# amin-abouee/semi-direct-visual-odometry

Hardware: AMD Instinct MI355X
Metric: frame-pair alignments/sec @2000 feats, 5-lvl pyramid; SE(3) err vs ref (higher is better)
Workload: dtype f64

## Files before the change

### semi-direct-visual-odometry_amd/csrc/align_refv.hip

```cpp
#include "svo_internal.h"
#include "svo_math.h"
#include "svo_wave.h"
#include "ref_common.h"

#include <utility>

namespace svo {
#if defined(SVO_TIMELINE)
SVO_TL_DEFINE(k2v)
SVO_TL_READER(k2v)
#endif


namespace {

using namespace refsel;

constexpr int kVT = 512;
constexpr int kVW = kVT / 64;
#ifndef SVO_ONEWAVE
#define SVO_ONEWAVE 2048
#endif
constexpr int kRowPad = 128;

#include "refv_rows.h"

template <class G, int R, uint32_t MB, bool PRE, uint32_t OW>
struct Lay {
    using Rows = G;
    static constexpr int kRows = R;
    static constexpr int kRegRows = G::kRegRows;
    static constexpr uint32_t kMbCap = MB;
    static constexpr bool kPreload = PRE;
    static constexpr uint32_t kCap = (uint32_t)R * kVT;
    static constexpr uint32_t kOneWave = OW;
    static constexpr uint32_t kStage = 2 * OW;
    static_assert(OW % 256 == 0 && OW / 64 <= G::kRegRows && OW <= 4096, "one-wave rows: register quads of wave 0");
    static_assert(R > G::kRegRows && R <= kRowPad, "rows");
    static_assert(2 * OW <= MB && MB % 64 == 0, "one-wave segment and its mailbox");
    static_assert(!PRE || kStage + 64 * G::kRegRows <= MB, "staging of wave 0's rows inside the mailbox");
    static_assert(!PRE || R % (kVW - 1) == 0, "stage_wave0 covers every row");
};
#ifndef SVO_ONEWAVE_A
#define SVO_ONEWAVE_A SVO_ONEWAVE
#endif
using LayA = Lay<RowsA, 98, 12288, true, SVO_ONEWAVE_A>;
using LayB = Lay<RowsB, 118, 4352, false, SVO_ONEWAVE>;
using LayC = Lay<RowsC, 128, 1344, false, 512>;
using LayADbg = Lay<RowsA, 98, 12288, true, 1024>;
using LayBDbg = Lay<RowsB, 118, 4352, false, 1024>;

template <class L>
struct VShared {
    double mbx[L::kMbCap + 64];
    uint32_t rec[4][kVW][kRowPad];
    uint32_t cnt[kVW][kRowPad];
    double pub[6];
    uint32_t pubk[4];
    double bcd;
    uint32_t srch[4];
    double lrow[L::kRows - L::kRegRows][kVT];
    uint32_t tmp[2 * kVW];
};
static_assert(sizeof(VShared<LayC>) <= 163840, "LayC's shared state fits the CU's LDS");

struct VDiag {
    uint32_t nblock[2], nwave[2], heap[2], nchunk[2];
    uint64_t cyc[2];
    uint64_t ph[12];
    uint32_t nlog;
#if defined(SVO_STAMPS_WAVES)
    union {
        uint32_t log[64][2];
        uint32_t phw[kVW][12];
    };
#else
    uint32_t log[64][2];
#endif
    double* tr;
    uint32_t trcap, ntr;
};
constexpr uint32_t kTrHead = 8;
#if defined(SVO_STAMPS_SMALL)
[[maybe_unused]] constexpr bool kStampsSmall = true;
#else
[[maybe_unused]] constexpr bool kStampsSmall = false;
#endif
#if defined(SVO_STAMPS) && defined(SVO_STAMPS_WAVES)
#define VSTAMP(i) \
    do { \
        if (kStampOn && dg) { \
            const uint64_t t_ = clock64(); \
            if (!kStampsSmall || small_round) phacc[i] += (uint32_t)(t_ - tstamp); \
            tstamp = t_; \
        } \
    } while (0)
#elif defined(SVO_STAMPS)
#define VSTAMP(i) \
    do { \
        if (kStampOn && dg && tid == 0) { \
            const uint64_t t_ = clock64(); \
            if (!kStampsSmall || small_round) dg->ph[i] += t_ - tstamp; \
            tstamp = t_; \
        } \
    } while (0)
#else
#define VSTAMP(i) \
    do { \
        (void)tstamp; \
    } while (0)
#endif

__device__ __forceinline__ uint32_t lane_sel(uint64_t m, uint32_t a, uint32_t b) {
    uint32_t r;
    asm("v_cndmask_b32_e64 %0, %2, %1, %3" : "=v"(r) : "v"(a), "v"(b), "s"(m));
    return r;
}
__device__ __forceinline__ uint32_t lane_put(uint32_t x, uint32_t v, uint32_t j, uint32_t me) {
    uint32_t r;
    uint64_t eq;
    asm("v_cmp_eq_u32_e64 %1, %2, %3\n\tv_cndmask_b32_e64 %0, %4, %5, %1"
        : "=v"(r), "=&s"(eq)
        : "v"(me), "s"(j), "v"(x), "v"(v));
    return r;
}
template <class L>
struct VSel {
    using G = typename L::Rows;
    static constexpr int R = L::kRows;
    static constexpr int kVRegRows = L::kRegRows;
    static constexpr int kGenQuads = G::kGenQuads;
    static constexpr uint32_t kMbCap = L::kMbCap;
    static constexpr uint32_t kOneWave = L::kOneWave;
    static constexpr uint32_t kStage = L::kStage;
    static constexpr int kQuads = (R + 3) / 4;
#ifndef SVO_FEWROWS
#define SVO_FEWROWS 8
#endif
    static constexpr int kFewRows = SVO_FEWROWS;
    static constexpr bool kChunkSteps = kMbCap < 12288;
#ifndef SVO_QG
#define SVO_QG 4
#endif
    static constexpr int kQG = SVO_QG;
    static constexpr bool kStampOn = L::kPreload;
    static __device__ __forceinline__ double vget(int r) { return G::vget(r); }
    static __device__ __forceinline__ void vset(int r, double x) { G::vset(r, x); }
    static __device__ __forceinline__ uint64_t vcmp_ge(int r, double p) { return G::vcmp_ge(r, p); }
    static __device__ __forceinline__ uint64_t vcmp_le(int r, double p) { return G::vcmp_le(r, p); }
    static __device__ __forceinline__ void vsel(int r, double x, uint64_t m) { G::vsel(r, x, m); }
    VShared<L>& sh;
    double* gseg;
    uint32_t gdummy;
    VDiag* dg;
    uint32_t M, nth;
    int tid, lane, wave;
    uint32_t f, l;
    uint32_t xk0 = 0, xk1 = 0;
    int depth;
    bool rec;
    double lo_val;
    int P;
    bool small_round = false;
#if defined(SVO_STAMPS) && defined(SVO_STAMPS_WAVES)
    uint32_t phacc[12] = {};
#endif

    template <bool kWrite, typename F>
    __device__ __forceinline__ void rows(int rlo, int rhi, F&& body) {
        const int r1 = rhi < kVRegRows - 1 ? rhi : kVRegRows - 1;
        for (int r = rlo; r <= r1; ++r) {
            double x = vget(r);
            body(r, x);
            if (kWrite) vset(r, x);
        }
#pragma unroll 2
        for (int r = rlo > kVRegRows ? rlo : kVRegRows; r <= rhi; ++r) {
            double& y = sh.lrow[r - kVRegRows][tid];
            double x = y;
            body(r, x);
            if (kWrite) y = x;
        }
    }
    __device__ __forceinline__ double row_val(int r) const {
        return r < kVRegRows ? vget(r) : sh.lrow[r - kVRegRows][tid];
    }
    __device__ __forceinline__ void row_set(int r, uint32_t ln, double x) {
        if ((uint32_t)lane != ln) return;
        if (r < kVRegRows) vset(r, x);
        else sh.lrow[r - kVRegRows][tid] = x;
    }
    __device__ __forceinline__ void load_raw(const double* src) {
        constexpr int kL = R - kVRegRows;
        if constexpr (kL <= 12) {
            double x[kL];
#pragma unroll
            for (int i = 0; i < kL; ++i) {
                const uint32_t q = (uint32_t)(kVRegRows + i) * kVT + (uint32_t)tid;
                x[i] = __builtin_nontemporal_load(src + (q < M ? q : 0u));
            }
            G::load(src, M * 8u, tid);
#pragma unroll
            for (int i = 0; i < kL; ++i) {
                const uint32_t q = (uint32_t)(kVRegRows + i) * kVT + (uint32_t)tid;
                sh.lrow[i][tid] = q < M ? x[i] : 0.0;
            }
        } else {
            G::load(src, M * 8u, tid);
#pragma unroll 2
            for (int r = kVRegRows; r < R; ++r) {
                const uint32_t q = (uint32_t)r * kVT + (uint32_t)tid;
                sh.lrow[r - kVRegRows][tid] = q < M ? src[q] : 0.0;
            }
        }
    }
    __device__ __forceinline__ void stage_wave0(const double* src) {
        double* const stg = sh.mbx + kStage;
#pragma unroll
        for (int i = 0; i < R / (kVW - 1); ++i) {
            const int r = wave - 1 + (kVW - 1) * i;
            const uint32_t q = (uint32_t)r * kVT + (uint32_t)lane;
            const double x = q < M ? src[q] : 0.0;
            if (r < kVRegRows) stg[64 * r + lane] = x;
            else sh.lrow[r - kVRegRows][lane] = x;
        }
    }
    __device__ __forceinline__ void unstage_wave0() {
        const uint32_t a = (uint32_t)(uintptr_t)(sh.mbx + kStage) + 8u * (uint32_t)lane;
        G::unstage(a);
    }
    __device__ __forceinline__ void load(const double* src, bool mad, double med, bool preloaded) {
        if (!preloaded) load_raw(src);
        if (mad) {
            const uint64_t mb = uni(__builtin_bit_cast(uint64_t, med));
            G::mad(mb);
            rows<true>(kVRegRows, R - 1, [&](int, double& x) __attribute__((always_inline)) { x = fabs(x - med); });
        }
    }
    __device__ __forceinline__ void wave_rows(uint32_t s0, uint32_t s1, int& rlo, int& rhi) const {
        const int w = wave;
        rlo = (int)s0 <= w ? 0 : ((int)s0 - w + kVW - 1) / kVW;
        rhi = (int)s1 < w ? -1 : ((int)s1 - w) / kVW;
    }
    static __device__ __forceinline__ uint64_t row_mask(int fw, int lw, int r) {
        const int b = r * kVT;
        const int lo = fw - b, hi = lw - b;
        return low_mask((uint32_t)(hi < 0 ? 0 : hi)) & ~low_mask((uint32_t)(lo < 0 ? 0 : lo));
    }
    __device__ __forceinline__ void publish(uint32_t q, int slot) {
        if (((q >> 6) & (kVW - 1)) != (uint32_t)wave) return;
        const double x = row_val((int)(q >> 9));
        if ((uint32_t)lane == (q & 63u)) sh.pub[slot] = x;
    }
    __device__ __forceinline__ void dump(double* dst, uint32_t dbase, double* dummy) {
        int rlo, rhi;
        wave_rows(f >> 6, (l - 1) >> 6, rlo, rhi);
        const int fo = (int)f - tid, lo = (int)l - tid;
        double* const d = dst + ((uint32_t)tid - dbase);
        double* const dl = dummy + lane;
        rows<false>(rlo, rhi, [&](int r, double x) __attribute__((always_inline)) {
            const int b = r * kVT;
            *(b >= fo && b < lo ? d + b : dl) = x;
        });
    }

    struct WaveRows {
        int rlo, rhi;
        uint64_t ge_first, le_first, last;
    };
    __device__ __forceinline__ WaveRows wave_segment(uint32_t s0, uint32_t s1) const {
        WaveRows w;
        wave_rows(s0, s1, w.rlo, w.rhi);
        const int fw = (int)f - 64 * wave, lw = (int)l - 64 * wave;
        w.le_first = row_mask(fw, lw, w.rlo);
        w.last = row_mask(fw, lw, w.rhi);
        const bool own_f = ((f >> 6) & (kVW - 1)) == (uint32_t)wave && (int)(f >> 9) == w.rlo;
        w.ge_first = w.le_first & ~(own_f ? 1ull << (f & 63u) : 0ull);
        return w;
    }
    static __device__ __forceinline__ void opaque(int& a, int& b) { asm volatile("" : "+s"(a), "+s"(b)); }
    template <int Q>
    __device__ __forceinline__ void cls_quad(double p, int rlo, int rhi, uint32_t (&acc)[2][4]) {
        opaque(rlo, rhi);
        if (4 * Q + 3 < rlo || 4 * Q > rhi) return;
        cls_quad_in<Q>(p, acc);
    }
    template <int Q>
    __device__ __forceinline__ void cls_quad_in(double p, uint32_t (&acc)[2][4]) {
        constexpr int g = (4 * Q) >> 6;
        if constexpr (Q < kGenQuads) {
            G::template cls4<Q>(p, acc[g]);
        } else {
#pragma unroll
            for (int i = 0; i < 4; ++i) {
                const int r = 4 * Q + i;
                if (r >= R) continue;
                const double x = sh.lrow[r - kVRegRows][tid];
                const uint64_t ge = __ballot(!(x < p)), le = __ballot(!(p < x));
                acc[g][0] = lane_write(acc[g][0], (uint32_t)ge, (uint32_t)(r & 63));
                acc[g][1] = lane_write(acc[g][1], (uint32_t)(ge >> 32), (uint32_t)(r & 63));
                acc[g][2] = lane_write(acc[g][2], (uint32_t)le, (uint32_t)(r & 63));
                acc[g][3] = lane_write(acc[g][3], (uint32_t)(le >> 32), (uint32_t)(r & 63));
            }
        }
    }
    template <int Gq, int... Is>
    __device__ __forceinline__ void cls_group(double p, int rlo, int rhi, uint32_t (&acc)[2][4],
                                              std::integer_sequence<int, Is...>) {
        opaque(rlo, rhi);
        constexpr int r0 = 4 * kQG * Gq, r1 = r0 + 4 * (int)sizeof...(Is) - 1;
        if (r1 < rlo || r0 > rhi) return;
        if (r0 >= rlo && r1 <= rhi) (cls_quad_in<kQG * Gq + Is>(p, acc), ...);
        else (cls_quad<kQG * Gq + Is>(p, rlo, rhi, acc), ...);
    }
    template <int... Gs>
    __device__ __forceinline__ void cls_quads(double p, int rlo, int rhi, uint32_t (&acc)[2][4],
                                              std::integer_sequence<int, Gs...>) {
        (cls_group<Gs>(p, rlo, rhi, acc, std::make_integer_sequence<int, (kQuads - kQG * Gs < kQG ? kQuads - kQG * Gs : kQG)>{}), ...);
    }
    __device__ __forceinline__ void cls_rows(double p, int rlo, int rhi, uint32_t (&acc)[2][4]) {
        for (int r = rlo; r <= rhi; ++r) {
            uint64_t ge, le;
            if (r < kVRegRows) {
                G::vcmp2(r, p, ge, le);
            } else {
                const double x = sh.lrow[r - kVRegRows][tid];
                ge = __ballot(!(x < p));
                le = __ballot(!(p < x));
            }
            const bool mine = lane == (r & 63);
#pragma unroll
            for (int g = 0; g < 2; ++g) {
                if (g != (r >> 6)) continue;
                acc[g][0] = mine ? (uint32_t)ge : acc[g][0];
// ... 52 lines not shown
                own += v < wave ? C.c[g][v] : 0u;
                t += C.c[g][v];
            }
            rt[g] = t;
            C.pw[g] = own;
        }
        const uint32_t i0 = wave_incl_scan(rt[0]);
        const uint32_t t0 = uni(lane_read(i0, 63));
        const uint32_t i1 = wave_incl_scan(rt[1]) + t0;
        C.rp[0] = i0 - rt[0];
        C.rp[1] = i1 - rt[1];
        C.pw[0] += C.rp[0];
        C.pw[1] += C.rp[1];
        const uint32_t tot = uni(lane_read(i1, 63));
        C.totG = tot & 0xFFFFu;
        C.totL = tot >> 16;
    }
    template <int G>
    __device__ __forceinline__ uint32_t step_pre_g(const Ctl& C, uint32_t ln, uint32_t v) const {
        uint32_t pk = uni(lane_read(C.rp[G], (int)ln));
#pragma unroll
        for (int u = 0; u < kVW; ++u)
            if ((uint32_t)u < v) pk += uni(lane_read(C.c[G][u], (int)ln));
        return pk;
    }
    __device__ __forceinline__ uint32_t step_pre(const Ctl& C, uint32_t s) const {
        const uint32_t r = s >> 3, v = s & (kVW - 1);
        return r < 64 ? step_pre_g<0>(C, r, v) : step_pre_g<1>(C, r - 64, v);
    }
    static __device__ __forceinline__ uint32_t kval(uint32_t pk, int kind) {
        return kind == 0 ? pk & 0xFFFFu : kind == 1 ? pk >> 16 : (pk & 0xFFFFu) + (pk >> 16);
    }
    template <int G>
    __device__ __forceinline__ uint32_t walk_row(const Ctl& C, uint32_t ln, int kind, uint32_t rank, uint32_t& pre) const {
        uint32_t pk = uni(lane_read(C.rp[G], (int)ln)), s = 0, p0 = pk;
#pragma unroll
        for (int u = 0; u < kVW; ++u) {
            if (kval(pk, kind) < rank) { s = (uint32_t)u; p0 = pk; }
            pk += uni(lane_read(C.c[G][u], (int)ln));
        }
        pre = p0;
        return (64u * G + ln) * kVW + s;
    }
    __device__ __forceinline__ uint32_t find_step(const Ctl& C, int kind, uint32_t rank, uint32_t& pre) const {
        const uint32_t n = popc(__ballot(kval(C.rp[0], kind) < rank)) + popc(__ballot(kval(C.rp[1], kind) < rank));
        const uint32_t jr = n - 1u;
        return jr < 64 ? walk_row<0>(C, jr, kind, rank, pre) : walk_row<1>(C, jr - 64, kind, rank, pre);
    }
    __device__ __forceinline__ uint64_t rec_mask(uint32_t s, int kind) const {
        const uint32_t r = s >> 3, v = s & (kVW - 1);
        return ((uint64_t)uni(sh.rec[2 * kind + 1][v][r]) << 32) | uni(sh.rec[2 * kind][v][r]);
    }
    __device__ __forceinline__ uint32_t locate(const Ctl& C, int kind, uint32_t rank) const {
        uint32_t pre;
        const uint32_t s = find_step(C, kind, rank, pre);
        return s * 64u + wave_select_bit(rec_mask(s, kind), rank - kval(pre, kind) - 1u);
    }
    __device__ __forceinline__ uint32_t locate_lds(const Ctl& C, int kind, uint32_t rank) const {
        const uint32_t n = popc(__ballot(kval(C.rp[0], kind) < rank)) + popc(__ballot(kval(C.rp[1], kind) < rank));
        const uint32_t jr = n - 1u, g = jr >> 6, ln = jr & 63u;
        uint32_t pk = uni(lane_read(g ? C.rp[1] : C.rp[0], (int)ln)), st = 0, p0 = pk;
#pragma unroll
        for (int u = 0; u < kVW; ++u) {
            if (kval(pk, kind) < rank) { st = (uint32_t)u; p0 = pk; }
            pk += uni(sh.cnt[u][jr]);
        }
        const uint32_t s = jr * kVW + st;
        return s * 64u + wave_select_bit(rec_mask(s, kind), rank - kval(p0, kind) - 1u);
    }
    __device__ __forceinline__ uint32_t wave_select_bit(uint64_t m, uint32_t j) const {
        const uint64_t hit = __ballot(((m >> lane) & 1ull) && lanes_below(m) == j);
        return (uint32_t)__builtin_ctzll(hit);
    }
    __device__ __forceinline__ uint32_t wave_crossing_ks(uint32_t gcar, uint32_t lcar, uint64_t ge, uint64_t le) const {
        const uint32_t me = (uint32_t)lane;
        const uint32_t g = gcar + lanes_below(ge) + (uint32_t)((ge >> me) & 1ull);
        const uint32_t lc = lcar - (lanes_below(le) + (uint32_t)((le >> me) & 1ull));
        const uint64_t q = __ballot(g >= lc);
        const uint32_t lo = q ? (uint32_t)__builtin_ctzll(q) + 1u : 64u;
        const uint32_t g1 = gcar + popc(ge & low_mask(lo - 1));
        const uint32_t l2 = lcar - popc(le & low_mask(lo));
        return g1 > l2 ? g1 : l2;
    }
    __device__ __forceinline__ void publish_cand(const Ctl& C, uint32_t q, int i, uint32_t ks, int side) {
        if (((q >> 6) & (kVW - 1)) != (uint32_t)wave) return;
        const double x = row_val((int)(q >> 9));
        uint32_t k = 0;
        if (ks) {
            const uint32_t s = q >> 6, b = q & 63u, r = s >> 3;
            const uint64_t m = rec_mask(s, side);
            if ((m >> b) & 1ull) {
                const uint32_t pp = r < 64 ? uni(lane_read(C.pw[0], (int)r)) : uni(lane_read(C.pw[1], (int)(r - 64)));
                const uint32_t below = popc(m & low_mask(b));
                k = side ? C.totL - ((pp >> 16) + below) : (pp & 0xFFFFu) + below + 1u;
                if (k > ks) k = 0;
            }
        }
        if ((uint32_t)lane == (q & 63u)) {
            sh.pub[i] = x;
            sh.pubk[i] = k;
        }
    }

    template <bool kWrite>
    __device__ __forceinline__ void generic_row(const Ctl& C, int side, int r, uint64_t gm, double p, uint32_t k0,
                                                uint32_t k1, bool chunked) {
        const uint32_t pp = r < 64 ? uni(lane_read(C.pw[0], r)) : uni(lane_read(C.pw[1], r - 64));
        const uint32_t nk = k1 - k0;
        const uint32_t b = side == 0 ? (pp & 0xFFFFu) - k0 : C.totL - 1u - k0 - (pp >> 16);
        double* const mbx = sh.mbx;
        const uint32_t dslot = kMbCap + (uint32_t)lane;
        uint64_t m;
        double x = 0.0;
        const bool reg = r < kVRegRows;
        if (!reg) x = sh.lrow[r - kVRegRows][tid];
        if (chunked) m = rec_mask((uint32_t)(r * kVW + wave), side);
        else if (side == 0) m = reg ? vcmp_ge(r, p) : __ballot(!(x < p));
        else m = reg ? vcmp_le(r, p) : __ballot(!(p < x));
        m &= gm;
        const uint32_t kk = side == 0 ? b + lanes_below(m) : b - lanes_below(m);
        const uint64_t okm = m & __ballot(kk < nk);
        const uint32_t a = lane_sel(okm, kk, dslot);
        if (kWrite) {
            mbx[a] = reg ? vget(r) : x;
        } else {
            const double t = mbx[a];
            if (reg) vsel(r, t, okm);
            else if ((okm >> lane) & 1ull) sh.lrow[r - kVRegRows][tid] = t;
        }
    }
    template <int Q, bool kWrite, int S>
    __device__ __forceinline__ void ex_quad(const Ctl& C, double p, int ra, int rb, const uint32_t (&pb)[2]) {
        opaque(ra, rb);
        if (4 * Q + 3 < ra || 4 * Q > rb) return;
        constexpr int g = (4 * Q) >> 6;
        if constexpr (Q < kGenQuads) {
            if (4 * Q >= ra && 4 * Q + 3 <= rb) {
                if (kWrite) G::template src4<Q, S>(p, pb[g]);
                else G::template tgt4<Q, S>(p, pb[g]);
            } else {
                if (kWrite) G::template src4e<Q, S>(p, pb[g], (uint32_t)ra, (uint32_t)(rb - ra));
                else G::template tgt4e<Q, S>(p, pb[g], (uint32_t)ra, (uint32_t)(rb - ra));
            }
        } else {
#pragma unroll
            for (int i = 0; i < 4; ++i) {
                const int r = 4 * Q + i;
                if (r < R && r >= ra && r <= rb) generic_row<kWrite>(C, S, r, ~0ull, p, xk0, xk1, false);
            }
        }
    }
    template <int Q, bool kWrite, int S>
    __device__ __forceinline__ void ex_quad_in(const Ctl& C, double p, const uint32_t (&pb)[2]) {
        constexpr int g = (4 * Q) >> 6;
        if constexpr (Q < kGenQuads) {
            if (kWrite) G::template src4<Q, S>(p, pb[g]);
            else G::template tgt4<Q, S>(p, pb[g]);
        } else {
#pragma unroll
            for (int i = 0; i < 4; ++i) {
                const int r = 4 * Q + i;
                if (r < R) generic_row<kWrite>(C, S, r, ~0ull, p, xk0, xk1, false);
            }
        }
    }
    template <bool kWrite, int S>
    __device__ __forceinline__ void ex_quads(const Ctl& C, double p, int ra, int rb, uint32_t k0) {
        const uint32_t mb = (uint32_t)(uintptr_t)sh.mbx - 8u * k0;
        uint32_t pb[2];
#pragma unroll
        for (int g = 0; g < 2; ++g)
            pb[g] = S == 0 ? mb + 8u * (C.pw[g] & 0xFFFFu) : mb + 8u * (C.totL - 1u - (C.pw[g] >> 16));
        ex_groups<kWrite, S>(C, p, ra, rb, pb, std::make_integer_sequence<int, (kQuads + kQG - 1) / kQG>{});
    }
    template <bool kWrite, int S, int Gq, int... Is>
    __device__ __forceinline__ void ex_group(const Ctl& C, double p, int ra, int rb, const uint32_t (&pb)[2],
                                             std::integer_sequence<int, Is...>) {
        opaque(ra, rb);
        constexpr int r0 = 4 * kQG * Gq, r1 = r0 + 4 * (int)sizeof...(Is) - 1;
        if (r1 < ra || r0 > rb) return;
        if (r0 >= ra && r1 <= rb) {
            if constexpr (!kWrite && G::kTgt8 && kQG == 4 && sizeof...(Is) == 4 && r1 < 4 * kGenQuads) {
                G::template tgt8<2 * Gq, S>(p, pb[r0 >> 6]);
                G::template tgt8<2 * Gq + 1, S>(p, pb[r0 >> 6]);
            } else {
                (ex_quad_in<kQG * Gq + Is, kWrite, S>(C, p, pb), ...);
            }
        }
        else (ex_quad<kQG * Gq + Is, kWrite, S>(C, p, ra, rb, pb), ...);
    }
    template <bool kWrite, int S, int... Gs>
    __device__ __forceinline__ void ex_groups(const Ctl& C, double p, int ra, int rb, const uint32_t (&pb)[2],
                                              std::integer_sequence<int, Gs...>) {
        (ex_group<kWrite, S, Gs>(C, p, ra, rb, pb,
                                 std::make_integer_sequence<int, (kQuads - kQG * Gs < kQG ? kQuads - kQG * Gs : kQG)>{}), ...);
    }
    template <bool kWrite>
    __device__ __forceinline__ void exchange(const Ctl& C, int side, uint32_t s0, uint32_t s1, uint32_t bstep, double p,
                                             uint32_t k0, uint32_t k1, bool chunked) {
        asm volatile("" : "+s"(s0), "+s"(s1));
        const WaveRows w = wave_segment(s0, s1);
        if (w.rlo > w.rhi) return;
        const uint64_t gfirst = side == 0 ? w.ge_first : w.le_first;
        if (chunked && !kChunkSteps) {
            for (int r = w.rlo; r <= w.rhi; ++r)
                generic_row<kWrite>(C, side, r, r == w.rlo ? gfirst : (r == w.rhi ? w.last : ~0ull), p, k0, k1, true);
            return;
        }
        generic_row<kWrite>(C, side, w.rlo, w.rlo == w.rhi ? gfirst & w.last : gfirst, p, k0, k1, chunked);
        if (w.rhi > w.rlo) generic_row<kWrite>(C, side, w.rhi, w.last, p, k0, k1, chunked);
        (void)bstep;
        const int ra = w.rlo + 1, rb = w.rhi - 1;
        if (ra > rb) return;
        if (rb - ra < kFewRows) {
            for (int r = ra; r <= rb; ++r) generic_row<kWrite>(C, side, r, ~0ull, p, k0, k1, false);
            return;
        }
        xk0 = k0;
        xk1 = k1;
        if (side == 0) ex_quads<kWrite, 0>(C, p, ra, rb, k0);
        else ex_quads<kWrite, 1>(C, p, ra, rb, k0);
    }

    __device__ __forceinline__ void refresh_ids() {
        asm volatile("" : "+v"(tid), "+v"(lane));
        wave = (int)uni((uint32_t)tid >> 6);
    }
    __device__ __forceinline__ bool tracing() const {
#if defined(SVO_STAMPS)
        return false;
#else
        return dg && dg->tr;
#endif
    }
    __device__ __forceinline__ double* trace_rec(uint32_t kind, uint32_t f0, uint32_t l0, double p, uint32_t ks,
                                                 uint32_t tg, uint32_t tl, uint32_t cut) {
        if (!tracing()) return nullptr;
        const uint32_t i = dg->ntr;
        if ((uint64_t)(i + 1u) * (kTrHead + M) > dg->trcap) return nullptr;
        double* const b = dg->tr + (uint64_t)i * (kTrHead + M);
        if (tid < (int)kTrHead) {
            const uint32_t j = (uint32_t)tid;
            const uint32_t u = j == 0 ? (uint32_t)(P + 10 * (int)kind) : j == 1 ? f0 : j == 2 ? l0 : j == 4 ? ks
                             : j == 5 ? tg : j == 6 ? tl : cut;
            b[j] = j == 3 ? p : (double)u;
        }
        return b + kTrHead;
    }
    __device__ __forceinline__ void trace_block(uint32_t f0, uint32_t l0, double p, uint32_t ks, uint32_t tg, uint32_t tl,
                                                uint32_t cut) {
        double* const v = trace_rec(0, f0, l0, p, ks, tg, tl, cut);
        if (v) {
            rows<false>(0, R - 1, [&](int r, double x) __attribute__((always_inline)) {
                const uint32_t q = (uint32_t)r * kVT + (uint32_t)tid;
                if (q < M) v[q] = x;
            });
        }
        __syncthreads();
        if (tracing() && tid == 0) ++dg->ntr;
        __syncthreads();
    }
    __device__ __forceinline__ void block_round(double p, uint32_t ch, double x0, double (&cand)[4]) {
        refresh_ids();
        uint64_t tstamp = dg ? clock64() : 0;
#if defined(SVO_STAMPS)
        const uint64_t tround = tstamp;
        const uint32_t S0 = l - f;
        small_round = S0 < 2048;
#endif
        classify(p, ch, x0);
        VSTAMP(1);
        __syncthreads();
        VSTAMP(2);
        Ctl C;
        counts(C);
        VSTAMP(8);
        const uint32_t totL = C.totL, totG = C.totG;
        uint32_t ks, lk1, rk, lk;
        auto search = [&](int which) __attribute__((always_inline)) {
            uint32_t pke;
            const uint32_t es = find_step(C, 2, totL, pke);
            const uint64_t mge = rec_mask(es, 0), mle = rec_mask(es, 1);
            ks = uni(wave_crossing_ks(pke & 0xFFFFu, totL - (pke >> 16), mge, mle));
            VSTAMP(9);
            const uint32_t ra = ks + 1u, rb = totL - ks + 1u, rc = ks;
            const uint32_t G0 = pke & 0xFFFFu, L0 = pke >> 16, cg = popc(mge), cl = popc(mle);
            const uint32_t ebase = es * 64u;
            if (which & 1)
                lk1 = ra > totG ? kNone
                      : (ra > G0 && ra <= G0 + cg) ? ebase + uni(wave_select_bit(mge, ra - G0 - 1u)) : uni(locate(C, 0, ra));
            if (which & 2)
                rk = ks == 0 ? kNone
                     : (rb > L0 && rb <= L0 + cl) ? ebase + uni(wave_select_bit(mle, rb - L0 - 1u)) : uni(locate(C, 1, rb));
            if (which & 4)
                lk = ks == 0 ? kNone
                     : (rc > G0 && rc <= G0 + cg) ? ebase + uni(wave_select_bit(mge, rc - G0 - 1u)) : uni(locate(C, 0, rc));
            VSTAMP(10);
        };
#if defined(SVO_K2V_ONECHAIN)
        if (wave == 0) {
            search(7);
            if (lane == 0) {
                sh.srch[0] = ks;
                sh.srch[1] = lk1;
                sh.srch[2] = rk;
                sh.srch[3] = lk;
            }
        }
        __syncthreads();
        ks = uni(sh.srch[0]);
        lk1 = uni(sh.srch[1]);
        rk = uni(sh.srch[2]);
        lk = uni(sh.srch[3]);
#elif !defined(SVO_K2V_ALLCHAINS)
        if (wave < 3) {
            search(1 << wave);
            if (lane == 0) {
                if (wave == 0) {
                    sh.srch[0] = ks;
                    sh.srch[1] = lk1;
                } else if (wave == 1) {
                    sh.srch[2] = rk;
                } else {
                    sh.srch[3] = lk;
                }
            }
        }
        __syncthreads();
        ks = uni(sh.srch[0]);
        lk1 = uni(sh.srch[1]);
        rk = uni(sh.srch[2]);
        lk = uni(sh.srch[3]);
#else
        search(7);
#endif
        const uint32_t cut = lk1 < rk ? lk1 : rk;
        const bool right = cut <= nth;
        const uint32_t nf = right ? cut : f, nl = right ? l : cut;
        const bool record = cut == nth && !rec;
        if (record) publish(lk == cut - 1u ? rk : cut - 1u, 4);
        const uint32_t nS = nl - nf;
        const bool need = nS > kOneWave && depth > 0;
        const uint32_t cq[4] = {nf + 1u, nf + nS / 2u, nl - 1u, nf};
        const int src_side = right ? 0 : 1, tgt_side = right ? 1 : 0;
        if (need) {
#pragma unroll
            for (int i = 0; i < 4; ++i) publish_cand(C, cq[i], i, ks, tgt_side);
        }
        const uint32_t sl = (l - 1) >> 6;
        const uint32_t s0L = f >> 6, s1L = lk != kNone ? lk >> 6 : 0u;
        const uint32_t s0R = rk != kNone ? rk >> 6 : sl + 1u, s1R = sl;
        const uint32_t nch = ks == 0 ? 1u : (ks + kMbCap - 1u) / kMbCap;
        uint32_t ck[4] = {0, 0, 0, 0};
        VSTAMP(3);
        auto chunk_steps = [&](int side, uint32_t k0, uint32_t k1, uint32_t& s0, uint32_t& s1) __attribute__((always_inline)) {
            if (side == 0) {
                s0 = uni(locate_lds(C, 0, k0 + 1u)) >> 6;
                s1 = uni(locate_lds(C, 0, k1)) >> 6;
            } else {
                s0 = uni(locate_lds(C, 1, C.totL - k1 + 1u)) >> 6;
                s1 = uni(locate_lds(C, 1, C.totL - k0)) >> 6;
            }
        };
        for (uint32_t it = 0; it < nch; ++it) {
            const uint32_t k0 = it * kMbCap, k1 = ks < k0 + kMbCap ? ks : k0 + kMbCap;
            if (ks) {
                if (kChunkSteps && nch > 1) {
                    uint32_t c0, c1;
                    chunk_steps(src_side, k0, k1, c0, c1);
                    if (src_side == 0) exchange<true>(C, 0, c0, c1, c1, p, k0, k1, true);
                    else exchange<true>(C, 1, c0, c1, c0, p, k0, k1, true);
                } else if (src_side == 0) {
                    exchange<true>(C, 0, s0L, s1L, s1L, p, k0, k1, nch > 1);
                } else {
                    exchange<true>(C, 1, s0R, s1R, s0R, p, k0, k1, nch > 1);
                }
            }
            VSTAMP(4);
            __syncthreads();
            VSTAMP(5);
            if (it == 0) {
                if (record) { lo_val = uni(sh.pub[4]); rec = true; }
                if (need) {
#pragma unroll
                    for (int i = 0; i < 4; ++i) {
                        cand[i] = uni(sh.pub[i]);
                        ck[i] = uni(sh.pubk[i]);
                    }
                }
            }
            if (ks) {
                if (kChunkSteps && nch > 1) {
                    uint32_t c0, c1;
                    chunk_steps(tgt_side, k0, k1, c0, c1);
                    if (tgt_side == 0) exchange<false>(C, 0, c0, c1, c1, p, k0, k1, true);
                    else exchange<false>(C, 1, c0, c1, c0, p, k0, k1, true);
                } else if (tgt_side == 0) {
                    exchange<false>(C, 0, s0L, s1L, s1L, p, k0, k1, nch > 1);
                } else {
                    exchange<false>(C, 1, s0R, s1R, s0R, p, k0, k1, nch > 1);
                }
                if (need) {
#pragma unroll
                    for (int i = 0; i < 4; ++i)
                        if (ck[i] > k0 && ck[i] <= k1) cand[i] = uni(sh.mbx[ck[i] - 1u - k0]);
                }
            }
            if (it + 1 < nch) __syncthreads();
        }
        if (nch > 1) __syncthreads();
        VSTAMP(6);
        if (dg && tid == 0) dg->nchunk[P] += nch > 1 ? 1u : 0u;
#if defined(SVO_STAMPS) && !defined(SVO_STAMPS_WAVES)
        if (kStampOn && dg && tid == 0 && dg->nlog < 64) {
            dg->log[dg->nlog][0] = S0;
            dg->log[dg->nlog][1] = (uint32_t)(clock64() - tround);
            ++dg->nlog;
        }
#endif
        if (tracing()) {
            const uint32_t f0 = f, l0 = l;
            f = nf;
            l = nl;
            trace_block(f0, l0, p, ks, totG, totL, cut);
        }
        f = nf;
        l = nl;
    }

    __device__ __forceinline__ double cand_at(uint32_t q) const {
        return uni(lane_read(vget((int)(q >> 6)), (int)(q & 63u)));
    }
    template <int Q>
    static __device__ __forceinline__ void w1_cls(double pe, uint32_t (&acc)[4], int js, int je) {
        if constexpr (Q < (int)(kOneWave / 256)) {
            if (js <= 4 * Q + 3 && je >= 4 * Q) G::template cls4<Q>(pe, acc);
            w1_cls<Q + 1>(pe, acc, js, je);
        }
    }
    template <int Q, int S, bool W>
    static __device__ __forceinline__ void w1_ex(uint32_t ml, uint32_t mh, uint32_t pkv, uint32_t ks, uint32_t tl1,
                                                 uint32_t mbb, int js, int je) {
        if constexpr (Q < (int)(kOneWave / 256)) {
            if (js <= 4 * Q + 3 && je >= 4 * Q) {
                if constexpr (W) G::template w1src<Q, S>(ml, mh, pkv, ks, tl1, mbb);
                else G::template w1tgt<Q, S>(ml, mh, pkv, ks, tl1, mbb);
            }
            w1_ex<Q + 1, S, W>(ml, mh, pkv, ks, tl1, mbb, js, je);
        }
    }
    __device__ __forceinline__ void wave_rounds(double* seg, double* mb, uint32_t& nrounds) {
        const uint32_t f0 = f, me = (uint32_t)lane;
        uint32_t fr = 0, lr = l - f;
        const uint32_t nrel = nth - f0;
#pragma unroll
        for (int j = 0; j < (int)(kOneWave / 64); ++j) vset(j, seg[64 * j + lane]);
        const uint32_t mbb = (uint32_t)(uintptr_t)mb;
        while (lr - fr > 64 && depth > 0) {
            --depth;
            ++nrounds;
            const uint32_t A = fr + 1, B = fr + (lr - fr) / 2, C = lr - 1;
            const double a = cand_at(A), b = cand_at(B), c = cand_at(C), xv = cand_at(fr);
            uint32_t chh;
            double pe;
            median3(a, b, c, A, B, C, chh, pe);
            vsel((int)(fr >> 6), pe, 1ull << (fr & 63u));
            vsel((int)(chh >> 6), xv, 1ull << (chh & 63u));
            int js = (int)(fr >> 6), je = (int)((lr - 1) >> 6);
            uint32_t acc[4] = {0, 0, 0, 0};
            opaque(js, je);
            w1_cls<0>(pe, acc, js, je);
            const bool live = (int)me >= js && (int)me <= je;
            const uint32_t rb0 = 64u * me;
            const uint32_t lo = fr > rb0 ? fr - rb0 : 0u;
            const uint32_t hi = live ? (lr - rb0 < 64u ? lr - rb0 : 64u) : 0u;
            const uint64_t inm = live ? low_mask(hi) & ~low_mask(lo) : 0ull;
            const uint64_t gem = inm & ~((int)me == js ? 1ull << (fr & 63u) : 0ull);
            acc[0] &= (uint32_t)gem;
            acc[1] &= (uint32_t)(gem >> 32);
            acc[2] &= (uint32_t)inm;
            acc[3] &= (uint32_t)(inm >> 32);
            const uint32_t cnt = ((uint32_t)__popc(acc[0]) + (uint32_t)__popc(acc[1])) |
                                 (((uint32_t)__popc(acc[2]) + (uint32_t)__popc(acc[3])) << 16);
            const uint32_t incl = wave_incl_scan(cnt);
            const uint32_t pkv = incl - cnt;
            const uint32_t tot = uni(lane_read(incl, 63));
            const uint32_t tG = tot & 0xFFFFu, tL = tot >> 16;
            const uint32_t gpl = pkv & 0xFFFFu, lpl = pkv >> 16;
            auto masks = [&](uint32_t jj, uint64_t& ge, uint64_t& le) __attribute__((always_inline)) {
                ge = ((uint64_t)uni(lane_read(acc[1], (int)jj)) << 32) | uni(lane_read(acc[0], (int)jj));
                le = ((uint64_t)uni(lane_read(acc[3], (int)jj)) << 32) | uni(lane_read(acc[2], (int)jj));
            };
            const uint64_t cq = __ballot(live && gpl + lpl < tL);
            const uint32_t jc = 63u - (uint32_t)__builtin_clzll(cq);
            uint64_t a0, b0m;
            masks(jc, a0, b0m);
            const uint32_t pkc = uni(lane_read(pkv, (int)jc));
            const uint32_t ks = uni(wave_crossing_ks(pkc & 0xFFFFu, tL - (pkc >> 16), a0, b0m));
            auto rank_pos = [&](int kind, uint32_t rank) __attribute__((always_inline)) -> uint32_t {
                if (rank == 0 || rank > (kind ? tL : tG)) return kNone;
                const uint64_t q = __ballot(live && (kind ? lpl : gpl) < rank);
                const uint32_t jj = 63u - (uint32_t)__builtin_clzll(q);
                const uint32_t pp = uni(lane_read(pkv, (int)jj));
                const uint32_t pre = kind ? pp >> 16 : pp & 0xFFFFu;
                uint64_t ge, le;
                masks(jj, ge, le);
                return 64u * jj + wave_select_bit(kind ? le : ge, rank - pre - 1u);
// ... 32 lines not shown
#pragma unroll
        for (int j = 0; j < (int)(kOneWave / 64); ++j) seg[64 * j + lane] = vget(j);
        if (lr - fr > 3 && depth > 0) row_rounds(seg, reinterpret_cast<uint32_t*>(mb), f0, fr, lr, nrounds);
        f = f0 + fr;
        l = f0 + lr;
    }
    __device__ __forceinline__ void row_rounds(double* seg, uint32_t* tab, uint32_t f0, uint32_t& fr, uint32_t& lr,
                                               uint32_t& nrounds) {
        const uint32_t me = (uint32_t)lane, w = fr, n0 = lr - fr;
        const uint32_t nr = nth - f0 - w;
        double x = seg[w + me];
        uint32_t a = 0, b = n0;
        while (b - a > 3 && depth > 0) {
            --depth;
            ++nrounds;
            const uint32_t A = a + 1, B = a + (b - a) / 2, C = b - 1;
            const double va = uni(lane_read(x, (int)A)), vb = uni(lane_read(x, (int)B)), vc = uni(lane_read(x, (int)C));
            const double x0 = uni(lane_read(x, (int)a));
            uint32_t ch;
            double pe;
            median3(va, vb, vc, A, B, C, ch, pe);
            x = me == a ? pe : (me == ch ? x0 : x);
            const bool live = me >= a && me < b;
            const uint64_t ge = __ballot(live && me != a && !(x < pe)), le = __ballot(live && !(pe < x));
            const uint32_t tG = popc(ge), tL = popc(le);
            const uint32_t ks = uni(wave_crossing_ks(0u, tL, ge, le));
            const uint32_t lk1 = ks + 1u <= tG ? uni(wave_select_bit(ge, ks)) : kNone;
            const uint32_t rk = ks >= 1u ? uni(wave_select_bit(le, tL - ks)) : kNone;
            const uint32_t cut = lk1 < rk ? lk1 : rk;
            if (cut == nr && !rec && nth >= 1u) {
                const uint32_t lk = ks >= 1u ? uni(wave_select_bit(ge, ks - 1u)) : kNone;
                lo_val = uni(lane_read(x, (int)(lk == cut - 1u ? rk : cut - 1u)));
                rec = true;
            }
            if (ks) {
                const uint32_t kg = lanes_below(ge) + 1u, kl = tL - lanes_below(le);
                const bool sg = ((ge >> me) & 1ull) && kg <= ks, sl = ((le >> me) & 1ull) && kl <= ks;
                if (sl) tab[kl - 1u] = me;
                if (sg) tab[64u + kg - 1u] = me;
                asm volatile("" ::: "memory");
                const uint32_t partner = sg ? tab[kg - 1u] : (sl ? tab[64u + kl - 1u] : me);
                const uint64_t u = __builtin_bit_cast(uint64_t, x);
                const uint32_t lo = (uint32_t)__builtin_amdgcn_ds_bpermute((int)(partner * 4u), (int)(uint32_t)u);
                const uint32_t hi = (uint32_t)__builtin_amdgcn_ds_bpermute((int)(partner * 4u), (int)(uint32_t)(u >> 32));
                x = __builtin_bit_cast(double, ((uint64_t)hi << 32) | lo);
                asm volatile("" ::: "memory");
            }
            if (tracing()) {
                double* const v = trace_rec(1, f0 + w + a, f0 + w + b, pe, ks, tG, tL, f0 + w + cut);
                if (v) {
                    if (me < n0) v[f0 + w + me] = x;
                    if (me == 0) ++dg->ntr;
                }
            }
            if (cut <= nr) a = cut;
            else b = cut;
        }
        if (me < n0) seg[w + me] = x;
        fr = w + a;
        lr = w + b;
    }
    __device__ __forceinline__ void select(const double* src, bool mad, double med, bool preloaded, bool preload_next,
                                           double& hi, double& lo, bool& did_preload, bool retire, bool& retired) {
        const uint64_t t0 = dg ? clock64() : 0;
        uint64_t tstamp = t0;
        did_preload = false;
        load(src, mad, med, preloaded);
        VSTAMP(0);
        f = 0;
        l = M;
        depth = M > 1 ? 2 * lg2(M) : 0;
        rec = false;
        lo_val = 0.0;
        double cand[4] = {0.0, 0.0, 0.0, 0.0};
        if (M >= 4) {
            const uint32_t qs[4] = {1u, M / 2u, M - 1u, 0u};
#pragma unroll
            for (int i = 0; i < 4; ++i) {
                const double x = src[qs[i]];
                cand[i] = uni(mad ? fabs(x - med) : x);
            }
        }
        uint32_t nblock = 0;
        while (l - f > kOneWave && depth > 0) {
            --depth;
            ++nblock;
            uint32_t ch;
            double p;
            median3(cand[0], cand[1], cand[2], f + 1u, f + (l - f) / 2u, l - 1u, ch, p);
            block_round(uni(p), uni(ch), cand[3], cand);
        }
        tstamp = dg ? clock64() : 0;
        __syncthreads();
        if (l - f > kOneWave) {
            dump(gseg, 0, gseg + gdummy);
            __threadfence_block();
            __syncthreads();
            if (tid == 0) {
                heap_select_at(gseg + f, l - f, nth + 1 - f, nth - f);
                hi = gseg[nth];
                lo = rec ? lo_val : (nth >= 1 ? gseg[nth - 1] : 0.0);
            }
            if (dg && tid == 0) dg->heap[P] = 1;
        } else {
            double* const seg = sh.mbx;
            const uint32_t f0 = f;
            dump(seg, f0, sh.mbx + kMbCap);
            __syncthreads();
#if !defined(SVO_K2V_KEEP_WAVES)
            if (retire && !preload_next && wave != 0) {
                retired = true;
                return;
            }
#endif
            did_preload = preload_next;
            if (preload_next && wave != 0) {
                load_raw(src);
                stage_wave0(src);
            }
            if (wave == 0) {
                uint32_t nw = 0;
                wave_rounds(seg, sh.mbx + kOneWave, nw);
                if (tid == 0) {
                    if (l - f <= 3) {
                        const uint32_t n = l - f;
                        double t[3] = {0.0, 0.0, 0.0};
                        for (uint32_t i = 0; i < n; ++i) t[i] = seg[f - f0 + i];
                        sort3(t, n);
                        hi = t[nth - f];
                        lo = rec ? lo_val : (nth >= f + 1 ? t[nth - 1 - f] : 0.0);
                    } else {
                        heap_select_at(seg + (f - f0), l - f, nth + 1 - f, nth - f);
                        hi = seg[nth - f0];
                        lo = rec ? lo_val : (nth >= f0 + 1 ? seg[nth - 1 - f0] : 0.0);
                        if (dg) dg->heap[P] = 1;
                    }
                    if (dg) dg->nwave[P] = nw;
                }
            }
        }
        __syncthreads();
        if (did_preload && wave == 0) unstage_wave0();
        VSTAMP(7);
#if defined(SVO_STAMPS) && defined(SVO_STAMPS_WAVES)
        if (kStampOn && dg && lane == 0) {
#pragma unroll
            for (int i = 0; i < 12; ++i) {
                dg->phw[wave][i] += phacc[i];
                if (tid == 0) dg->ph[i] += phacc[i];
                phacc[i] = 0;
            }
        }
#endif
        if (dg && tid == 0) {
            dg->nblock[P] = nblock;
            dg->cyc[P] = clock64() - t0;
        }
    }
};

template <class L, bool kRetire>
__device__ __forceinline__ void refv_robust_scale(const double* src, VShared<L>& sh, double* gseg, VDiag* dg, uint32_t M,
                                                  uint32_t n, double& med, double& mad) {
    L::Rows::fence();
    VSel<L> s{sh, gseg, (uint32_t)((M + 63u) / 64u * 64u), dg};
    s.M = M;
    s.nth = n / 2;
    s.tid = (int)threadIdx.x;
    s.lane = s.tid & 63;
    s.wave = (int)uni((uint32_t)(s.tid >> 6));
    const bool even = (M & 1u) == 0 && s.nth >= 1;
    double m0 = 0.0;
    bool pre = false;
    for (int P = 0; P < 2; ++P) {
        s.P = P;
        double lo = 0.0, hi = 0.0;
        bool did = false, retired = false;
        s.select(src, P == 1, m0, pre, P == 0 && L::kPreload, hi, lo, did, kRetire && P == 1, retired);
        if (retired) return;
        pre = did;
        if (s.tid == 0) sh.bcd = even ? (lo + hi) / 2.0 : hi;
        __syncthreads();
        const double r = uni(sh.bcd);
        __syncthreads();
        if (P == 0) m0 = r;
        else mad = r;
    }
    med = m0;
}

template <class L>
__device__ __forceinline__ void scale_refv_pair(const AlignArgs& a, VShared<L>& sh) {
    const int pair = blockIdx.x, tid = threadIdx.x, lane = tid & 63, wave = tid >> 6;
    PairState& S = a.state[pair];
    if (!S.active) return;
    const PairDesc& P = a.pairs[pair];
    const int nf = P.n_ref + P.n_kf;
    const uint32_t M = (uint32_t)nf * (uint32_t)a.area;
    const uint8_t* __restrict__ fvis = a.fvis + (int64_t)pair * a.max_f;
    uint32_t nrv = 0, ncv = 0;
    for (int f = tid; f < nf; f += kVT) {
        const uint8_t v = fvis[f];
        nrv += v & 1;
        ncv += v >> 1;
    }
    nrv = wave_sum_u(nrv);
    ncv = wave_sum_u(ncv);
    if (lane == 0) { sh.tmp[wave] = nrv; sh.tmp[kVW + wave] = ncv; }
    __syncthreads();
    nrv = 0; ncv = 0;
    for (int w = 0; w < kVW; ++w) { nrv += sh.tmp[w]; ncv += sh.tmp[kVW + w]; }
    const uint32_t n = ncv * (uint32_t)a.area;
    double med = kDblMax, mad = 0.0;
    if (n > 0)
        refv_robust_scale<L, true>(a.scratch + (int64_t)pair * a.key_stride, sh,
                             reinterpret_cast<double*>(a.sel + (int64_t)pair * a.sel_stride), nullptr, M, n, med, mad);
    if (tid == 0) {
        double sigma = 1.482602218505602 * mad;
        if (sigma <= 2.220446049250313e-16) sigma = 2.220446049250313e-16;
        S.med = med;
        S.mad = mad;
        S.sigma = sigma;
        S.c = 4.6851 * sigma;
        S.n = n;
        S.n_ref_vis = nrv;
        S.scale_kernel = SVO_SCALE_K2V;
    }
}

}

template <class L>
__global__ void __launch_bounds__(kVT, 1) align_scale_refv_kernel(AlignArgs a, int level) {
    __shared__ VShared<L> sh;
    (void)level;
    SVO_TL_SCOPE(k2v, kTlK2V, level, a.pair_base);
    scale_refv_pair<L>(a, sh);
}
// ... 78 lines not shown
```

Measured before the change: 189,500.

## Add LDS-resident mid-size selection phase between block rounds and one-wave rounds

Adds a mid-size phase for layout A. Once the active segment fits in 7168 elements, it is dumped into the shared-memory mailbox, and partition rounds classify and exchange directly against LDS instead of the per-thread register/LDS row arrays. This cuts the per-round cost of touching all 98 rows and the chunked mailbox exchange for medium segments, and uses batched loads. It adds complexity: a second exchange path, index rebasing (moff, nth adjustments) and an extra compaction copy before the one-wave stage.

```diff
diff --git a/semi-direct-visual-odometry_amd/csrc/align_refv.hip b/semi-direct-visual-odometry_amd/csrc/align_refv.hip
--- a/semi-direct-visual-odometry_amd/csrc/align_refv.hip
+++ b/semi-direct-visual-odometry_amd/csrc/align_refv.hip
@@ -25,7 +25,7 @@
 
 #include "refv_rows.h"
 
-template <class G, int R, uint32_t MB, bool PRE, uint32_t OW>
+template <class G, int R, uint32_t MB, bool PRE, uint32_t OW, uint32_t MID = 0>
 struct Lay {
     using Rows = G;
     static constexpr int kRows = R;
@@ -35,6 +35,13 @@
     static constexpr uint32_t kCap = (uint32_t)R * kVT;
     static constexpr uint32_t kOneWave = OW;
     static constexpr uint32_t kStage = 2 * OW;
+    static constexpr uint32_t kMid = MID;
+#ifndef SVO_MID_BATCH
+#define SVO_MID_BATCH 4
+#endif
+    static constexpr int kMidBatch = OW >= 2048 ? SVO_MID_BATCH : 1;
+    static_assert(MID == 0 || (MID % kVT == 0 && MID > OW && MID / kVT <= 64 && MID + MID / 2 <= MB),
+                  "mid-size segment and its mailbox inside the mailbox array");
     static_assert(OW % 256 == 0 && OW / 64 <= G::kRegRows && OW <= 4096, "one-wave rows: register quads of wave 0");
     static_assert(R > G::kRegRows && R <= kRowPad, "rows");
     static_assert(2 * OW <= MB && MB % 64 == 0, "one-wave segment and its mailbox");
@@ -44,10 +51,13 @@
 #ifndef SVO_ONEWAVE_A
 #define SVO_ONEWAVE_A SVO_ONEWAVE
 #endif
-using LayA = Lay<RowsA, 98, 12288, true, SVO_ONEWAVE_A>;
+#ifndef SVO_MID
+#define SVO_MID 7168
+#endif
+using LayA = Lay<RowsA, 98, 12288, true, SVO_ONEWAVE_A, SVO_MID>;
 using LayB = Lay<RowsB, 118, 4352, false, SVO_ONEWAVE>;
 using LayC = Lay<RowsC, 128, 1344, false, 512>;
-using LayADbg = Lay<RowsA, 98, 12288, true, 1024>;
+using LayADbg = Lay<RowsA, 98, 12288, true, 1024, SVO_MID>;
 using LayBDbg = Lay<RowsB, 118, 4352, false, 1024>;
 
 template <class L>
@@ -133,6 +143,9 @@
     static constexpr uint32_t kMbCap = L::kMbCap;
     static constexpr uint32_t kOneWave = L::kOneWave;
     static constexpr uint32_t kStage = L::kStage;
+    static constexpr uint32_t kMid = L::kMid;
+    static constexpr int kMidRows = (int)(kMid / kVT);
+    static constexpr int kMidBatch = L::kMidBatch;
     static constexpr int kQuads = (R + 3) / 4;
 #ifndef SVO_FEWROWS
 #define SVO_FEWROWS 8
@@ -162,6 +175,7 @@
     double lo_val;
     int P;
     bool small_round = false;
+    uint32_t moff = 0, mlen = 0;
 #if defined(SVO_STAMPS) && defined(SVO_STAMPS_WAVES)
     uint32_t phacc[12] = {};
 #endif
@@ -247,9 +261,10 @@
         const int lo = fw - b, hi = lw - b;
         return low_mask((uint32_t)(hi < 0 ? 0 : hi)) & ~low_mask((uint32_t)(lo < 0 ? 0 : lo));
     }
+    template <bool kM = false>
     __device__ __forceinline__ void publish(uint32_t q, int slot) {
         if (((q >> 6) & (kVW - 1)) != (uint32_t)wave) return;
-        const double x = row_val((int)(q >> 9));
+        const double x = kM ? sh.mbx[(q & ~(uint32_t)(kVT - 1)) + (uint32_t)tid] : row_val((int)(q >> 9));
         if ((uint32_t)lane == (q & 63u)) sh.pub[slot] = x;
     }
     __device__ __forceinline__ void dump(double* dst, uint32_t dbase, double* dummy) {
@@ -468,9 +483,10 @@
         const uint32_t l2 = lcar - popc(le & low_mask(lo));
         return g1 > l2 ? g1 : l2;
     }
+    template <bool kM = false>
     __device__ __forceinline__ void publish_cand(const Ctl& C, uint32_t q, int i, uint32_t ks, int side) {
         if (((q >> 6) & (kVW - 1)) != (uint32_t)wave) return;
-        const double x = row_val((int)(q >> 9));
+        const double x = kM ? sh.mbx[(q & ~(uint32_t)(kVT - 1)) + (uint32_t)tid] : row_val((int)(q >> 9));
         uint32_t k = 0;
         if (ks) {
             const uint32_t s = q >> 6, b = q & 63u, r = s >> 3;
@@ -566,7 +582,12 @@
         constexpr int r0 = 4 * kQG * Gq, r1 = r0 + 4 * (int)sizeof...(Is) - 1;
         if (r1 < ra || r0 > rb) return;
         if (r0 >= ra && r1 <= rb) {
-            if constexpr (!kWrite && G::kTgt8 && kQG == 4 && sizeof...(Is) == 4 && r1 < 4 * kGenQuads) {
+#if defined(SVO_STAMPS)
+            constexpr bool kUse8 = false;
+#else
+            constexpr bool kUse8 = G::kTgt8;
+#endif
+            if constexpr (!kWrite && kUse8 && kQG == 4 && sizeof...(Is) == 4 && r1 < 4 * kGenQuads) {
                 G::template tgt8<2 * Gq, S>(p, pb[r0 >> 6]);
                 G::template tgt8<2 * Gq + 1, S>(p, pb[r0 >> 6]);
             } else {
@@ -608,6 +629,79 @@
         else ex_quads<kWrite, 1>(C, p, ra, rb, k0);
     }
 
+    __device__ __forceinline__ void classify_mid(double p, uint32_t ch, double x0, uint32_t (&acc)[4]) {
+        double* const A = sh.mbx;
+        if ((f & (uint32_t)(kVT - 1)) == (uint32_t)tid) A[f] = p;
+        if ((ch & (uint32_t)(kVT - 1)) == (uint32_t)tid) A[ch] = x0;
+        const WaveRows w = wave_segment(f >> 6, (l - 1) >> 6);
+        const int r0 = (int)(f >> 9), r1 = (int)((l - 1) >> 9);
+        acc[0] = acc[1] = acc[2] = acc[3] = 0;
+#pragma unroll
+        for (int g = 0; g < (kMidRows + kMidBatch - 1) / kMidBatch; ++g) {
+            if (kMidBatch * g + kMidBatch - 1 < r0 || kMidBatch * g > r1) continue;
+            double x[kMidBatch];
+#pragma unroll
+            for (int i = 0; i < kMidBatch; ++i)
+                if (kMidBatch * g + i < kMidRows) x[i] = A[kVT * (kMidBatch * g + i) + tid];
+#pragma unroll
+            for (int i = 0; i < kMidBatch; ++i) {
+                const int j = kMidBatch * g + i;
+                if (j >= kMidRows) continue;
+                const uint64_t ge = __ballot(!(x[i] < p)), le = __ballot(!(p < x[i]));
+                acc[0] = lane_write(acc[0], (uint32_t)ge, (uint32_t)j);
+                acc[1] = lane_write(acc[1], (uint32_t)(ge >> 32), (uint32_t)j);
+                acc[2] = lane_write(acc[2], (uint32_t)le, (uint32_t)j);
+                acc[3] = lane_write(acc[3], (uint32_t)(le >> 32), (uint32_t)j);
+            }
+        }
+        const int j = lane;
+        const bool in = j >= w.rlo && j <= w.rhi;
+        uint64_t gm = in ? ~0ull : 0ull, lm = gm;
+        if (j == w.rlo) { gm &= w.ge_first; lm &= w.le_first; }
+        if (j == w.rhi) { gm &= w.last; lm &= w.last; }
+        acc[0] &= (uint32_t)gm;
+        acc[1] &= (uint32_t)(gm >> 32);
+        acc[2] &= (uint32_t)lm;
+        acc[3] &= (uint32_t)(lm >> 32);
+#pragma unroll
+        for (int c = 0; c < 4; ++c) sh.rec[c][wave][j] = acc[c];
+        sh.cnt[wave][j] = (__popc(acc[0]) + __popc(acc[1])) | ((__popc(acc[2]) + __popc(acc[3])) << 16);
+    }
+    template <bool kWrite>
+    __device__ __forceinline__ void exchange_mid(const Ctl& C, const uint32_t (&acc)[4], int side, uint32_t ks, int ra,
+                                                 int rb) {
+        double* const A = sh.mbx;
+        double* const mb = sh.mbx + kMid;
+        const uint32_t dslot = kMbCap - kMid + (uint32_t)lane;
+        const uint32_t ml = side == 0 ? acc[0] : acc[2], mh = side == 0 ? acc[1] : acc[3];
+#pragma unroll
+        for (int g = 0; g < (kMidRows + kMidBatch - 1) / kMidBatch; ++g) {
+            if (kMidBatch * g + kMidBatch - 1 < ra || kMidBatch * g > rb) continue;
+            uint32_t a[kMidBatch];
+            uint64_t okm[kMidBatch];
+            double t[kMidBatch];
+#pragma unroll
+            for (int i = 0; i < kMidBatch; ++i) {
+                const int j = kMidBatch * g + i;
+                if (j >= kMidRows) continue;
+                const uint64_t m = ((uint64_t)uni(lane_read(mh, j)) << 32) | uni(lane_read(ml, j));
+                const uint32_t pp = uni(lane_read(C.pw[0], j));
+                const uint32_t b = side == 0 ? (pp & 0xFFFFu) : C.totL - 1u - (pp >> 16);
+                const uint32_t kk = side == 0 ? b + lanes_below(m) : b - lanes_below(m);
+                okm[i] = m & __ballot(kk < ks);
+                a[i] = lane_sel(okm[i], kk, dslot);
+                t[i] = kWrite ? A[kVT * j + tid] : mb[a[i]];
+            }
+#pragma unroll
+            for (int i = 0; i < kMidBatch; ++i) {
+                const int j = kMidBatch * g + i;
+                if (j >= kMidRows) continue;
+                if (kWrite) mb[a[i]] = t[i];
+                else if ((okm[i] >> lane) & 1ull) A[kVT * j + tid] = t[i];
+            }
+        }
+    }
+
     __device__ __forceinline__ void refresh_ids() {
         asm volatile("" : "+v"(tid), "+v"(lane));
         wave = (int)uni((uint32_t)tid >> 6);
@@ -646,6 +740,21 @@
         if (tracing() && tid == 0) ++dg->ntr;
         __syncthreads();
     }
+    __device__ __forceinline__ void trace_mid(uint32_t f0, uint32_t l0, double p, uint32_t ks, uint32_t tg, uint32_t tl,
+                                              uint32_t cut) {
+        double* const v = trace_rec(2, moff + f0, moff + l0, p, ks, tg, tl, moff + cut);
+        if (v) {
+#pragma unroll
+            for (int j = 0; j < kMidRows; ++j) {
+                const uint32_t i = (uint32_t)(kVT * j + tid);
+                if (i < mlen) v[moff + i] = sh.mbx[i];
+            }
+        }
+        __syncthreads();
+        if (tracing() && tid == 0) ++dg->ntr;
+        __syncthreads();
+    }
+    template <bool kM = false>
     __device__ __forceinline__ void block_round(double p, uint32_t ch, double x0, double (&cand)[4]) {
         refresh_ids();
         uint64_t tstamp = dg ? clock64() : 0;
@@ -654,7 +763,9 @@
         const uint32_t S0 = l - f;
         small_round = S0 < 2048;
 #endif
-        classify(p, ch, x0);
+        [[maybe_unused]] uint32_t macc[4];
+        if constexpr (kM) classify_mid(p, ch, x0, macc);
+        else classify(p, ch, x0);
         VSTAMP(1);
         __syncthreads();
         VSTAMP(2);
@@ -724,19 +835,19 @@
         const bool right = cut <= nth;
         const uint32_t nf = right ? cut : f, nl = right ? l : cut;
         const bool record = cut == nth && !rec;
-        if (record) publish(lk == cut - 1u ? rk : cut - 1u, 4);
+        if (record) publish<kM>(lk == cut - 1u ? rk : cut - 1u, 4);
         const uint32_t nS = nl - nf;
         const bool need = nS > kOneWave && depth > 0;
         const uint32_t cq[4] = {nf + 1u, nf + nS / 2u, nl - 1u, nf};
         const int src_side = right ? 0 : 1, tgt_side = right ? 1 : 0;
         if (need) {
 #pragma unroll
-            for (int i = 0; i < 4; ++i) publish_cand(C, cq[i], i, ks, tgt_side);
+            for (int i = 0; i < 4; ++i) publish_cand<kM>(C, cq[i], i, ks, tgt_side);
         }
         const uint32_t sl = (l - 1) >> 6;
         const uint32_t s0L = f >> 6, s1L = lk != kNone ? lk >> 6 : 0u;
         const uint32_t s0R = rk != kNone ? rk >> 6 : sl + 1u, s1R = sl;
-        const uint32_t nch = ks == 0 ? 1u : (ks + kMbCap - 1u) / kMbCap;
+        const uint32_t nch = kM || ks == 0 ? 1u : (ks + kMbCap - 1u) / kMbCap;
         uint32_t ck[4] = {0, 0, 0, 0};
         VSTAMP(3);
         auto chunk_steps = [&](int side, uint32_t k0, uint32_t k1, uint32_t& s0, uint32_t& s1) __attribute__((always_inline)) {
@@ -750,7 +861,12 @@
         };
         for (uint32_t it = 0; it < nch; ++it) {
             const uint32_t k0 = it * kMbCap, k1 = ks < k0 + kMbCap ? ks : k0 + kMbCap;
-            if (ks) {
+            if constexpr (kM) {
+                if (ks) {
+                    if (src_side == 0) exchange_mid<true>(C, macc, 0, ks, (int)(f >> 9), (int)(lk >> 9));
+                    else exchange_mid<true>(C, macc, 1, ks, (int)(rk >> 9), (int)((l - 1) >> 9));
+                }
+            } else if (ks) {
                 if (kChunkSteps && nch > 1) {
                     uint32_t c0, c1;
                     chunk_steps(src_side, k0, k1, c0, c1);
@@ -775,7 +891,17 @@
                     }
                 }
             }
-            if (ks) {
+            if constexpr (kM) {
+                if (ks) {
+                    if (tgt_side == 0) exchange_mid<false>(C, macc, 0, ks, (int)(f >> 9), (int)(lk >> 9));
+                    else exchange_mid<false>(C, macc, 1, ks, (int)(rk >> 9), (int)((l - 1) >> 9));
+                    if (need) {
+#pragma unroll
+                        for (int i = 0; i < 4; ++i)
+                            if (ck[i] > 0) cand[i] = uni(sh.mbx[kMid + ck[i] - 1u]);
+                    }
+                }
+            } else if (ks) {
                 if (kChunkSteps && nch > 1) {
                     uint32_t c0, c1;
                     chunk_steps(tgt_side, k0, k1, c0, c1);
@@ -799,7 +925,7 @@
         if (dg && tid == 0) dg->nchunk[P] += nch > 1 ? 1u : 0u;
 #if defined(SVO_STAMPS) && !defined(SVO_STAMPS_WAVES)
         if (kStampOn && dg && tid == 0 && dg->nlog < 64) {
-            dg->log[dg->nlog][0] = S0;
+            dg->log[dg->nlog][0] = S0 | (kM ? 0x80000000u : 0u);
             dg->log[dg->nlog][1] = (uint32_t)(clock64() - tround);
             ++dg->nlog;
         }
@@ -808,7 +934,8 @@
             const uint32_t f0 = f, l0 = l;
             f = nf;
             l = nl;
-            trace_block(f0, l0, p, ks, totG, totL, cut);
+            if constexpr (kM) trace_mid(f0, l0, p, ks, totG, totL, cut);
+            else trace_block(f0, l0, p, ks, totG, totL, cut);
         }
         f = nf;
         l = nl;
@@ -1007,7 +1134,8 @@
             }
         }
         uint32_t nblock = 0;
-        while (l - f > kOneWave && depth > 0) {
+        constexpr uint32_t kBlockMin = kMid > 0 ? kMid : kOneWave;
+        while (l - f > kBlockMin && depth > 0) {
             --depth;
             ++nblock;
             uint32_t ch;
@@ -1017,8 +1145,49 @@
         }
         tstamp = dg ? clock64() : 0;
         __syncthreads();
+        bool in_mid = false;
+        if constexpr (kMid > 0) in_mid = l - f > kOneWave && depth > 0;
+        uint32_t nmid = 0;
+        if (in_mid) {
+            moff = f;
+            mlen = l - f;
+            dump(sh.mbx, moff, sh.mbx + kMbCap);
+#pragma unroll
+            for (int c = 0; c < 4; ++c) sh.rec[c][wave][64 + lane] = 0;
+            sh.cnt[wave][64 + lane] = 0;
+            f = 0;
+            l = mlen;
+            nth -= moff;
+            __syncthreads();
+            while (l - f > kOneWave && depth > 0) {
+                --depth;
+                ++nmid;
+                uint32_t ch;
+                double p;
+                median3(cand[0], cand[1], cand[2], f + 1u, f + (l - f) / 2u, l - 1u, ch, p);
+                block_round<true>(uni(p), uni(ch), cand[3], cand);
+            }
+            __syncthreads();
+            if (l - f > kOneWave) {
+                for (uint32_t i = f + (uint32_t)tid; i < l; i += kVT) gseg[moff + i] = sh.mbx[i];
+            } else {
+                constexpr int kN = (int)(kOneWave / kVT);
+                double t[kN];
+#pragma unroll
+                for (int j = 0; j < kN; ++j) {
+                    const uint32_t i = f + (uint32_t)(kVT * j + tid);
+                    t[j] = sh.mbx[i < kMid ? i : 0u];
+                }
+                __syncthreads();
+#pragma unroll
+                for (int j = 0; j < kN; ++j) sh.mbx[kVT * j + tid] = t[j];
+            }
+            f += moff;
+            l += moff;
+            nth += moff;
+        }
         if (l - f > kOneWave) {
-            dump(gseg, 0, gseg + gdummy);
+            if (!in_mid) dump(gseg, 0, gseg + gdummy);
             __threadfence_block();
             __syncthreads();
             if (tid == 0) {
@@ -1030,7 +1199,7 @@
         } else {
             double* const seg = sh.mbx;
             const uint32_t f0 = f;
-            dump(seg, f0, sh.mbx + kMbCap);
+            if (!in_mid) dump(seg, f0, sh.mbx + kMbCap);
             __syncthreads();
 #if !defined(SVO_K2V_KEEP_WAVES)
             if (retire && !preload_next && wave != 0) {
@@ -1078,7 +1247,7 @@
         }
 #endif
         if (dg && tid == 0) {
-            dg->nblock[P] = nblock;
+            dg->nblock[P] = nblock | (nmid << 16);
             dg->cyc[P] = clock64() - t0;
         }
     }
```

Result: faster. 193,800 (median of 6 runs) (+2.3%).
